# mit-han-lab/duo-attention

Measured on NVIDIA H100. Metric: decode tok/s @512K ctx (+ prefill tok/s @128K in `prefill`), Llama-3-8B, DuoAttention 50% retrieval heads, higher is better.
Workload: dtype bf16

## Files before the change

### duo_attention_b200/csrc/attn_tc.cu

```cuda
#include <cstdlib>

#include "duo_common.cuh"

namespace duo {

constexpr int TC_THREADS = 384;
constexpr int TC_TILE = 128;
constexpr int TC_BOX_BYTES = TC_TILE * 128;
constexpr int TC_TILE_BYTES = 2 * TC_BOX_BYTES;
constexpr int TC_MAX_W = kTcMaxWindow;
constexpr int TC_SMEM_BYTES = 5 * TC_TILE_BYTES + TC_MAX_W + 1024;

struct TcParams {
  void* out;
  long long out_batch_stride;
  int q_len, n_q_heads, group, n_full, n_stream, batch;
  int sink, recent, W;
  long long full_len, total, lo;
  float scale_log2;
  int cache_scan;
  int n_tok_tiles;
  int seq_rank, seq_world, seq_block;
  float* part_o;
  float* part_lse;
};

__device__ __forceinline__ void wg_fence() { asm volatile("wgmma.fence.sync.aligned;" ::: "memory"); }
__device__ __forceinline__ void wg_commit() { asm volatile("wgmma.commit_group.sync.aligned;" ::: "memory"); }
template <int N>
__device__ __forceinline__ void wg_wait() {
  asm volatile("wgmma.wait_group.sync.aligned %0;" ::"n"(N) : "memory");
}
__device__ __forceinline__ void wg_fence_regs(float (&d)[64]) {
#pragma unroll
  for (int i = 0; i < 64; ++i) asm volatile("" : "+f"(d[i])::"memory");
}

__device__ __forceinline__ uint64_t make_smem_desc(uint32_t saddr, uint32_t lbo_bytes, uint32_t sbo_bytes) {
  uint64_t d = 0;
  d |= (uint64_t)((saddr >> 4) & 0x3FFF);
  d |= (uint64_t)((lbo_bytes >> 4) & 0x3FFF) << 16;
  d |= (uint64_t)((sbo_bytes >> 4) & 0x3FFF) << 32;
  d |= 1ull << 62;
  return d;
}

template <bool BF16>
__device__ __forceinline__ void wgmma_ss(float (&d)[64], uint64_t adesc, uint64_t bdesc, uint32_t accum) {
  if constexpr (BF16) {
    asm volatile(
        "{\n\t.reg .pred p;\n\tsetp.ne.b32 p, %66, 0;\n\t"
        "wgmma.mma_async.sync.aligned.m64n128k16.f32.bf16.bf16 {%0,%1,%2,%3,%4,%5,%6,%7,%8,%9,%10,%11,%12,%13,%14,%15,%16,%17,%18,%19,%20,%21,%22,%23,%24,%25,%26,%27,%28,%29,%30,%31,%32,%33,%34,%35,%36,%37,%38,%39,%40,%41,%42,%43,%44,%45,%46,%47,%48,%49,%50,%51,%52,%53,%54,%55,%56,%57,%58,%59,%60,%61,%62,%63}, %64, %65, p, 1, 1, 0, 0;\n\t}"
        : "+f"(d[0]), "+f"(d[1]), "+f"(d[2]), "+f"(d[3]), "+f"(d[4]), "+f"(d[5]), "+f"(d[6]), "+f"(d[7]), "+f"(d[8]), "+f"(d[9]), "+f"(d[10]), "+f"(d[11]), "+f"(d[12]), "+f"(d[13]), "+f"(d[14]), "+f"(d[15]), "+f"(d[16]), "+f"(d[17]), "+f"(d[18]), "+f"(d[19]), "+f"(d[20]), "+f"(d[21]), "+f"(d[22]), "+f"(d[23]), "+f"(d[24]), "+f"(d[25]), "+f"(d[26]), "+f"(d[27]), "+f"(d[28]), "+f"(d[29]), "+f"(d[30]), "+f"(d[31]), "+f"(d[32]), "+f"(d[33]), "+f"(d[34]), "+f"(d[35]), "+f"(d[36]), "+f"(d[37]), "+f"(d[38]), "+f"(d[39]), "+f"(d[40]), "+f"(d[41]), "+f"(d[42]), "+f"(d[43]), "+f"(d[44]), "+f"(d[45]), "+f"(d[46]), "+f"(d[47]), "+f"(d[48]), "+f"(d[49]), "+f"(d[50]), "+f"(d[51]), "+f"(d[52]), "+f"(d[53]), "+f"(d[54]), "+f"(d[55]), "+f"(d[56]), "+f"(d[57]), "+f"(d[58]), "+f"(d[59]), "+f"(d[60]), "+f"(d[61]), "+f"(d[62]), "+f"(d[63])
        : "l"(adesc), "l"(bdesc), "r"(accum));
  } else {
    asm volatile(
        "{\n\t.reg .pred p;\n\tsetp.ne.b32 p, %66, 0;\n\t"
        "wgmma.mma_async.sync.aligned.m64n128k16.f32.f16.f16 {%0,%1,%2,%3,%4,%5,%6,%7,%8,%9,%10,%11,%12,%13,%14,%15,%16,%17,%18,%19,%20,%21,%22,%23,%24,%25,%26,%27,%28,%29,%30,%31,%32,%33,%34,%35,%36,%37,%38,%39,%40,%41,%42,%43,%44,%45,%46,%47,%48,%49,%50,%51,%52,%53,%54,%55,%56,%57,%58,%59,%60,%61,%62,%63}, %64, %65, p, 1, 1, 0, 0;\n\t}"
        : "+f"(d[0]), "+f"(d[1]), "+f"(d[2]), "+f"(d[3]), "+f"(d[4]), "+f"(d[5]), "+f"(d[6]), "+f"(d[7]), "+f"(d[8]), "+f"(d[9]), "+f"(d[10]), "+f"(d[11]), "+f"(d[12]), "+f"(d[13]), "+f"(d[14]), "+f"(d[15]), "+f"(d[16]), "+f"(d[17]), "+f"(d[18]), "+f"(d[19]), "+f"(d[20]), "+f"(d[21]), "+f"(d[22]), "+f"(d[23]), "+f"(d[24]), "+f"(d[25]), "+f"(d[26]), "+f"(d[27]), "+f"(d[28]), "+f"(d[29]), "+f"(d[30]), "+f"(d[31]), "+f"(d[32]), "+f"(d[33]), "+f"(d[34]), "+f"(d[35]), "+f"(d[36]), "+f"(d[37]), "+f"(d[38]), "+f"(d[39]), "+f"(d[40]), "+f"(d[41]), "+f"(d[42]), "+f"(d[43]), "+f"(d[44]), "+f"(d[45]), "+f"(d[46]), "+f"(d[47]), "+f"(d[48]), "+f"(d[49]), "+f"(d[50]), "+f"(d[51]), "+f"(d[52]), "+f"(d[53]), "+f"(d[54]), "+f"(d[55]), "+f"(d[56]), "+f"(d[57]), "+f"(d[58]), "+f"(d[59]), "+f"(d[60]), "+f"(d[61]), "+f"(d[62]), "+f"(d[63])
        : "l"(adesc), "l"(bdesc), "r"(accum));
  }
}
template <bool BF16>
__device__ __forceinline__ void wgmma_rs(float (&d)[64], const uint32_t* a, uint64_t bdesc) {
  if constexpr (BF16) {
    asm volatile(
        "{\n\t.reg .pred p;\n\tsetp.ne.b32 p, %69, 0;\n\t"
        "wgmma.mma_async.sync.aligned.m64n128k16.f32.bf16.bf16 {%0,%1,%2,%3,%4,%5,%6,%7,%8,%9,%10,%11,%12,%13,%14,%15,%16,%17,%18,%19,%20,%21,%22,%23,%24,%25,%26,%27,%28,%29,%30,%31,%32,%33,%34,%35,%36,%37,%38,%39,%40,%41,%42,%43,%44,%45,%46,%47,%48,%49,%50,%51,%52,%53,%54,%55,%56,%57,%58,%59,%60,%61,%62,%63}, {%64, %65, %66, %67}, %68, p, 1, 1, 1;\n\t}"
        : "+f"(d[0]), "+f"(d[1]), "+f"(d[2]), "+f"(d[3]), "+f"(d[4]), "+f"(d[5]), "+f"(d[6]), "+f"(d[7]), "+f"(d[8]), "+f"(d[9]), "+f"(d[10]), "+f"(d[11]), "+f"(d[12]), "+f"(d[13]), "+f"(d[14]), "+f"(d[15]), "+f"(d[16]), "+f"(d[17]), "+f"(d[18]), "+f"(d[19]), "+f"(d[20]), "+f"(d[21]), "+f"(d[22]), "+f"(d[23]), "+f"(d[24]), "+f"(d[25]), "+f"(d[26]), "+f"(d[27]), "+f"(d[28]), "+f"(d[29]), "+f"(d[30]), "+f"(d[31]), "+f"(d[32]), "+f"(d[33]), "+f"(d[34]), "+f"(d[35]), "+f"(d[36]), "+f"(d[37]), "+f"(d[38]), "+f"(d[39]), "+f"(d[40]), "+f"(d[41]), "+f"(d[42]), "+f"(d[43]), "+f"(d[44]), "+f"(d[45]), "+f"(d[46]), "+f"(d[47]), "+f"(d[48]), "+f"(d[49]), "+f"(d[50]), "+f"(d[51]), "+f"(d[52]), "+f"(d[53]), "+f"(d[54]), "+f"(d[55]), "+f"(d[56]), "+f"(d[57]), "+f"(d[58]), "+f"(d[59]), "+f"(d[60]), "+f"(d[61]), "+f"(d[62]), "+f"(d[63])
        : "r"(a[0]), "r"(a[1]), "r"(a[2]), "r"(a[3]), "l"(bdesc), "r"(1));
  } else {
    asm volatile(
        "{\n\t.reg .pred p;\n\tsetp.ne.b32 p, %69, 0;\n\t"
        "wgmma.mma_async.sync.aligned.m64n128k16.f32.f16.f16 {%0,%1,%2,%3,%4,%5,%6,%7,%8,%9,%10,%11,%12,%13,%14,%15,%16,%17,%18,%19,%20,%21,%22,%23,%24,%25,%26,%27,%28,%29,%30,%31,%32,%33,%34,%35,%36,%37,%38,%39,%40,%41,%42,%43,%44,%45,%46,%47,%48,%49,%50,%51,%52,%53,%54,%55,%56,%57,%58,%59,%60,%61,%62,%63}, {%64, %65, %66, %67}, %68, p, 1, 1, 1;\n\t}"
        : "+f"(d[0]), "+f"(d[1]), "+f"(d[2]), "+f"(d[3]), "+f"(d[4]), "+f"(d[5]), "+f"(d[6]), "+f"(d[7]), "+f"(d[8]), "+f"(d[9]), "+f"(d[10]), "+f"(d[11]), "+f"(d[12]), "+f"(d[13]), "+f"(d[14]), "+f"(d[15]), "+f"(d[16]), "+f"(d[17]), "+f"(d[18]), "+f"(d[19]), "+f"(d[20]), "+f"(d[21]), "+f"(d[22]), "+f"(d[23]), "+f"(d[24]), "+f"(d[25]), "+f"(d[26]), "+f"(d[27]), "+f"(d[28]), "+f"(d[29]), "+f"(d[30]), "+f"(d[31]), "+f"(d[32]), "+f"(d[33]), "+f"(d[34]), "+f"(d[35]), "+f"(d[36]), "+f"(d[37]), "+f"(d[38]), "+f"(d[39]), "+f"(d[40]), "+f"(d[41]), "+f"(d[42]), "+f"(d[43]), "+f"(d[44]), "+f"(d[45]), "+f"(d[46]), "+f"(d[47]), "+f"(d[48]), "+f"(d[49]), "+f"(d[50]), "+f"(d[51]), "+f"(d[52]), "+f"(d[53]), "+f"(d[54]), "+f"(d[55]), "+f"(d[56]), "+f"(d[57]), "+f"(d[58]), "+f"(d[59]), "+f"(d[60]), "+f"(d[61]), "+f"(d[62]), "+f"(d[63])
        : "r"(a[0]), "r"(a[1]), "r"(a[2]), "r"(a[3]), "l"(bdesc), "r"(1));
  }
}

template <typename T>
struct TcType;
template <>
struct TcType<__nv_bfloat16> {
  static constexpr bool bf16 = true;
  __device__ static uint32_t pack(float a, float b) {
    __nv_bfloat162 v = __floats2bfloat162_rn(a, b);
    return *reinterpret_cast<uint32_t*>(&v);
  }
};
template <>
struct TcType<__half> {
  static constexpr bool bf16 = false;
  __device__ static uint32_t pack(float a, float b) {
    __half2 v = __floats2half2_rn(a, b);
    return *reinterpret_cast<uint32_t*>(&v);
  }
};

struct TcBarriers {
  uint64_t q_full;
  uint64_t k_full[2], k_empty[2], v_full[2], v_empty[2];
};

template <typename T, bool SEQ = false, bool SHARE = false, bool RAGGED = false>
__global__ void __launch_bounds__(TC_THREADS, 1)
duo_attn_tc_kernel(const __grid_constant__ CUtensorMap map_q, const __grid_constant__ CUtensorMap map_fk,
                   const __grid_constant__ CUtensorMap map_fv, const __grid_constant__ CUtensorMap map_rk,
                   const __grid_constant__ CUtensorMap map_rv, const TcParams p,
                   const __grid_constant__ CUtensorMap map_pk, const __grid_constant__ CUtensorMap map_pv,
                   const long long share_len, const __grid_constant__ RaggedChunks rc) {
  static_assert(!(SEQ && SHARE), "a shared prefix is not sequence-sharded");
  static_assert(!(RAGGED && (SEQ || SHARE)), "a ragged prefill reads sharing from row_share, and is not sharded");
  extern __shared__ __align__(1024) uint8_t smem_raw[];
  uint8_t* smem = reinterpret_cast<uint8_t*>((reinterpret_cast<uintptr_t>(smem_raw) + 1023) & ~uintptr_t(1023));
  __shared__ TcBarriers bars;

  uint8_t* sQ = smem;
  uint8_t* sK = smem + 1 * TC_TILE_BYTES;
  uint8_t* sV = smem + 3 * TC_TILE_BYTES;
  uint8_t* sValid = smem + 5 * TC_TILE_BYTES;

  const int tid = threadIdx.x;
  const int b = blockIdx.y;

  int x = blockIdx.x;
  const int per_kvh = p.group * p.n_tok_tiles;
  const int kvh = x / per_kvh;
  x -= kvh * per_kvh;
  const int qh = kvh * p.group + x / p.n_tok_tiles;
  int q_len = p.q_len, n_tok_tiles = p.n_tok_tiles, cache_scan = p.cache_scan, q_off = 0, donor = -1;
  long long full_len = p.full_len, total = p.total, lo = p.lo, pre_len = 0;
  if constexpr (RAGGED) {
    q_len = rc.len[b];
    n_tok_tiles = (q_len + TC_TILE - 1) / TC_TILE;
    if (x % p.n_tok_tiles >= n_tok_tiles) return;
    q_off = rc.off[b];
    full_len = rc.row_state[4 * b];
    total = rc.row_state[4 * b + 1];
    lo = rc.row_state[4 * b + 2];
    cache_scan = (int)min((long long)p.W, total);
    pre_len = ragged_chunk_share(rc, b, donor);
  }
  const int tok0 = (n_tok_tiles - 1 - (x % p.n_tok_tiles)) * TC_TILE;
  const bool is_full = kvh < p.n_full;
  const int tok_hi = min(q_len, tok0 + TC_TILE);
  long long a0 = 0, a1, b0 = 0, b1 = 0, base;
  if (is_full) {
    base = full_len;
    a1 = full_len + tok_hi;
    if constexpr (SEQ) a1 = seq_local_len(a1, p.seq_rank, p.seq_world, p.seq_block);
  } else {
    base = p.W;
    a1 = cache_scan;
    b0 = p.W;
    b1 = (long long)p.W + tok_hi;
  }
  const int nA = (int)((a1 - a0 + TC_TILE - 1) / TC_TILE);
  const int nB = (int)((b1 - b0 + TC_TILE - 1) / TC_TILE);
  const int n_tiles = nA + nB;
  const CUtensorMap* mk = is_full ? &map_fk : &map_rk;
  const CUtensorMap* mv = is_full ? &map_fv : &map_rv;
  const int head_coord = is_full ? (b * p.n_full + kvh) : (b * p.n_stream + (kvh - p.n_full));
  auto tile_start = [&](int i) -> long long {
    return i < nA ? a0 + (long long)i * TC_TILE : b0 + (long long)(i - nA) * TC_TILE;
  };

  if (tid == 0) {
    prefetch_tmap(&map_q);
    prefetch_tmap(mk);
    prefetch_tmap(mv);
    if constexpr (SHARE) {
      if (is_full) {
        prefetch_tmap(&map_pk);
        prefetch_tmap(&map_pv);
      }
    }
    mbar_init(&bars.q_full, 1);
    for (int s = 0; s < 2; ++s) {
      mbar_init(&bars.k_full[s], 1);
      mbar_init(&bars.k_empty[s], 256);
      mbar_init(&bars.v_full[s], 1);
      mbar_init(&bars.v_empty[s], 256);
    }
    fence_barrier_init();
  }
  if (!is_full) {
    for (int j = tid; j < p.W; j += TC_THREADS) sValid[j] = stream_slot_valid(j, p.sink, p.recent, total, lo) ? 1 : 0;
  }
  __syncthreads();

  if (tid < 128) {
    asm volatile("setmaxnreg.dec.sync.aligned.u32 24;");
    if constexpr (SEQ) {
      if (n_tiles == 0) return;
    }
    if (tid == 0) {
      mbar_expect_tx(&bars.q_full, TC_TILE_BYTES);
      const int q_row = RAGGED ? q_off + tok0 : tok0, q_b = RAGGED ? 0 : b;
      tma_load_3d(sQ, &map_q, &bars.q_full, qh * kHeadDim, q_row, q_b);
      tma_load_3d(sQ + TC_BOX_BYTES, &map_q, &bars.q_full, qh * kHeadDim + 64, q_row, q_b);
      for (int j = 0; j < n_tiles; ++j) {
        const int st = j & 1;
        const uint32_t ph = (j >> 1) & 1;
        if constexpr (RAGGED) {
          const long long t0 = tile_start(j);
          int r0 = (int)t0, hc = head_coord;
          if (is_full && rc.row_geom) {
            const bool pre = t0 < pre_len;
            r0 = (int)(pre ? ragged_pool_row(rc, donor, p.n_full, kvh, t0) : ragged_pool_row(rc, b, p.n_full, kvh, t0 - pre_len));
            hc = 0;
          }
          mbar_wait(&bars.k_empty[st], ph ^ 1);
          mbar_expect_tx(&bars.k_full[st], TC_TILE_BYTES);
          tma_load_3d(sK + st * TC_TILE_BYTES, mk, &bars.k_full[st], 0, r0, hc);
          tma_load_3d(sK + st * TC_TILE_BYTES + TC_BOX_BYTES, mk, &bars.k_full[st], 64, r0, hc);
          mbar_wait(&bars.v_empty[st], ph ^ 1);
          mbar_expect_tx(&bars.v_full[st], TC_TILE_BYTES);
          tma_load_3d(sV + st * TC_TILE_BYTES, mv, &bars.v_full[st], 0, r0, hc);
          tma_load_3d(sV + st * TC_TILE_BYTES + TC_BOX_BYTES, mv, &bars.v_full[st], 64, r0, hc);
          continue;
        }
        if constexpr (SHARE) {
          const long long t0 = tile_start(j);
          const bool pre = is_full && t0 < share_len;
          const CUtensorMap* tk = pre ? &map_pk : mk;
          const CUtensorMap* tv = pre ? &map_pv : mv;
          const int r0 = (int)(is_full && !pre ? t0 - share_len : t0);
          mbar_wait(&bars.k_empty[st], ph ^ 1);
          mbar_expect_tx(&bars.k_full[st], TC_TILE_BYTES);
          tma_load_3d(sK + st * TC_TILE_BYTES, tk, &bars.k_full[st], 0, r0, head_coord);
          tma_load_3d(sK + st * TC_TILE_BYTES + TC_BOX_BYTES, tk, &bars.k_full[st], 64, r0, head_coord);
          mbar_wait(&bars.v_empty[st], ph ^ 1);
          mbar_expect_tx(&bars.v_full[st], TC_TILE_BYTES);
          tma_load_3d(sV + st * TC_TILE_BYTES, tv, &bars.v_full[st], 0, r0, head_coord);
          tma_load_3d(sV + st * TC_TILE_BYTES + TC_BOX_BYTES, tv, &bars.v_full[st], 64, r0, head_coord);
          continue;
        }
        const int j0 = (int)tile_start(j);
        mbar_wait(&bars.k_empty[st], ph ^ 1);
        mbar_expect_tx(&bars.k_full[st], TC_TILE_BYTES);
        tma_load_3d(sK + st * TC_TILE_BYTES, mk, &bars.k_full[st], 0, j0, head_coord);
        tma_load_3d(sK + st * TC_TILE_BYTES + TC_BOX_BYTES, mk, &bars.k_full[st], 64, j0, head_coord);
        mbar_wait(&bars.v_empty[st], ph ^ 1);
        mbar_expect_tx(&bars.v_full[st], TC_TILE_BYTES);
        tma_load_3d(sV + st * TC_TILE_BYTES, mv, &bars.v_full[st], 0, j0, head_coord);
        tma_load_3d(sV + st * TC_TILE_BYTES + TC_BOX_BYTES, mv, &bars.v_full[st], 64, j0, head_coord);
      }
    }
    return;
  }

  asm volatile("setmaxnreg.inc.sync.aligned.u32 240;");
  constexpr bool kBf16 = TcType<T>::bf16;
  const int wg = (tid >> 7) - 1;
  const int wt = tid & 127;
  const int quad = wt & 3;
  const int row0 = wg * 64 + (wt >> 5) * 16 + ((wt & 31) >> 2);
  const float c = p.scale_log2;
  long long min_limit = base + tok0 + wg * 64;
  int tok[2];
  bool row_ok[2];
  long long limit[2];
#pragma unroll
  for (int i = 0; i < 2; ++i) {
    tok[i] = tok0 + row0 + 8 * i;
    row_ok[i] = tok[i] < q_len;
    limit[i] = base + tok[i];
  }
  auto seq_last_key = [&](int t) { return seq_local_len(p.full_len + t + 1, p.seq_rank, p.seq_world, p.seq_block) - 1; };
  if constexpr (SEQ) {
    if (is_full) {
      min_limit = seq_last_key(tok0 + wg * 64);
#pragma unroll
      for (int i = 0; i < 2; ++i) limit[i] = seq_last_key(tok[i]);
    }
  }

  const uint32_t q_addr = smem_u32(sQ) + wg * 64 * 128, k_addr = smem_u32(sK), v_addr = smem_u32(sV);
  auto issue_s = [&](float (&s)[64], int st) {
    const uint32_t ka = k_addr + st * TC_TILE_BYTES;
#pragma unroll
    for (int kk = 0; kk < 8; ++kk) {
      const uint32_t off = (kk >> 2) * TC_BOX_BYTES + (kk & 3) * 32;
      wgmma_ss<kBf16>(s, make_smem_desc(q_addr + off, 16, 1024), make_smem_desc(ka + off, 16, 1024), kk > 0);
    }
  };
  auto issue_pv = [&](float (&o)[64], const uint32_t (&pk)[32], int st) {
    const uint32_t va = v_addr + st * TC_TILE_BYTES;
#pragma unroll
    for (int kk = 0; kk < 8; ++kk) wgmma_rs<kBf16>(o, &pk[4 * kk], make_smem_desc(va + kk * 2048, TC_BOX_BYTES, 1024));
  };

  float s[64], o[64];
#pragma unroll
  for (int i = 0; i < 64; ++i) o[i] = 0.f;
  float m_run[2] = {-INFINITY, -INFINITY};
  float l_run[2] = {0.f, 0.f};

  auto store_partial = [&](int i, float inv, float l) {
    if (!row_ok[i]) return;
    const long long row = ((long long)b * p.q_len + tok[i]) * p.n_q_heads + qh;
#pragma unroll
    for (int nb = 0; nb < 16; ++nb)
      *reinterpret_cast<float2*>(p.part_o + row * kHeadDim + nb * 8 + quad * 2) =
          make_float2(o[nb * 4 + 2 * i] * inv, o[nb * 4 + 2 * i + 1] * inv);
    if (quad == 0) p.part_lse[row] = l > 0.f ? m_run[i] * c + log2f(l) : -INFINITY;
  };
  if constexpr (SEQ) {
    if (n_tiles == 0) {
      store_partial(0, 0.f, 0.f);
      store_partial(1, 0.f, 0.f);
      return;
    }
  }
  mbar_wait(&bars.q_full, 0);
  mbar_wait(&bars.k_full[0], 0);
  wg_fence();
  issue_s(s, 0);
  wg_commit();
  wg_wait<0>();
  wg_fence_regs(s);
  mbar_arrive(&bars.k_empty[0]);

  for (int j = 0; j < n_tiles; ++j) {
    const int st = j & 1;
    const uint32_t ph = (j >> 1) & 1;
    const long long j0 = tile_start(j);
    const long long jend = (j < nA) ? a1 : b1;
    const bool cache_seg = (!is_full) && (j < nA);
    const bool need_mask = cache_seg || (j0 + TC_TILE > jend) || (j0 + TC_TILE - 1 > min_limit);
    if (need_mask) {
#pragma unroll
      for (int nb = 0; nb < 16; ++nb) {
#pragma unroll
        for (int e = 0; e < 2; ++e) {
          const long long jj = j0 + nb * 8 + quad * 2 + e;
          bool slot_ok = jj < jend;
          if (cache_seg) slot_ok = slot_ok && (jj < p.W) && (sValid[jj < p.W ? jj : 0] != 0);
#pragma unroll
          for (int i = 0; i < 2; ++i)
            if (!(slot_ok && row_ok[i] && jj <= limit[i])) s[nb * 4 + 2 * i + e] = -INFINITY;
        }
      }
    }
    uint32_t pk[32];
#pragma unroll
    for (int i = 0; i < 2; ++i) {
      float mx = -INFINITY;
#pragma unroll
      for (int nb = 0; nb < 16; ++nb) mx = fmaxf(mx, fmaxf(s[nb * 4 + 2 * i], s[nb * 4 + 2 * i + 1]));
      mx = fmaxf(mx, __shfl_xor_sync(0xffffffffu, mx, 1));
      mx = fmaxf(mx, __shfl_xor_sync(0xffffffffu, mx, 2));
      const float m_new = fmaxf(m_run[i], mx);
      const float alpha = (m_new == -INFINITY) ? 1.f : fast_exp2((m_run[i] - m_new) * c);
      const float mref_c = (m_new == -INFINITY) ? 0.f : m_new * c;
      m_run[i] = m_new;
      float rs = 0.f;
#pragma unroll
      for (int nb = 0; nb < 16; ++nb) {
        const float p0 = fast_exp2(__fmaf_rn(s[nb * 4 + 2 * i], c, -mref_c));
        const float p1 = fast_exp2(__fmaf_rn(s[nb * 4 + 2 * i + 1], c, -mref_c));
        rs += p0 + p1;
        pk[nb * 2 + i] = TcType<T>::pack(p0, p1);
        o[nb * 4 + 2 * i] *= alpha;
        o[nb * 4 + 2 * i + 1] *= alpha;
      }
      l_run[i] = l_run[i] * alpha + rs;
    }
    mbar_wait_spin(&bars.v_full[st], ph);
    wg_fence();
    issue_pv(o, pk, st);
    wg_commit();
    const bool more = j + 1 < n_tiles;
    if (more) {
      const int st1 = (j + 1) & 1;
      mbar_wait_spin(&bars.k_full[st1], ((j + 1) >> 1) & 1);
      wg_fence();
      issue_s(s, st1);
      wg_commit();
    }
    wg_wait<0>();
    wg_fence_regs(o);
    wg_fence_regs(s);
    mbar_arrive(&bars.v_empty[st]);
    if (more) mbar_arrive(&bars.k_empty[(j + 1) & 1]);
  }

  if constexpr (SEQ) {
    if (is_full) {
#pragma unroll
      for (int i = 0; i < 2; ++i) {
        float l = l_run[i];
        l += __shfl_xor_sync(0xffffffffu, l, 1);
        l += __shfl_xor_sync(0xffffffffu, l, 2);
        store_partial(i, l > 0.f ? 1.f / l : 0.f, l);
      }
      return;
    }
  }
  T* out_b = reinterpret_cast<T*>(p.out) + (RAGGED ? (long long)q_off * p.n_q_heads * kHeadDim : (long long)b * p.out_batch_stride);
#pragma unroll
  for (int i = 0; i < 2; ++i) {
    float l = l_run[i];
    l += __shfl_xor_sync(0xffffffffu, l, 1);
    l += __shfl_xor_sync(0xffffffffu, l, 2);
    const float inv = l > 0.f ? 1.f / l : 0.f;
    if (row_ok[i]) {
      T* dst = out_b + ((long long)tok[i] * p.n_q_heads + qh) * kHeadDim + quad * 2;
#pragma unroll
      for (int nb = 0; nb < 16; ++nb)
        *reinterpret_cast<uint32_t*>(dst + nb * 8) = TcType<T>::pack(o[nb * 4 + 2 * i] * inv, o[nb * 4 + 2 * i + 1] * inv);
    }
  }
}

typedef CUresult (*EncodeTiledFn)(CUtensorMap*, CUtensorMapDataType, cuuint32_t, void*, const cuuint64_t*,
                                  const cuuint64_t*, const cuuint32_t*, const cuuint32_t*, CUtensorMapInterleave,
                                  CUtensorMapSwizzle, CUtensorMapL2promotion, CUtensorMapFloatOOBfill);
EncodeTiledFn get_encode_fn();

bool tc_prefill_supported(const duo_layer* L, const duo_cache_state* st, int q_len) {
  (void)st;
  if (L->d.kv_format != DUO_KV_SAME) return false;
  if (q_len < TC_TILE) return false;
  if (L->d.sink + L->d.recent > TC_MAX_W) return false;
  return true;
}

template <bool SEQ, bool SHARE = false>
static int launch_tc(const duo_layer* L, const duo_cache_state* st, const void* q, long long q_row_stride, void* out,
                     float* part_o, float* part_lse, int q_len, float scale, cudaStream_t stream,
                     const duo_layer* prefix = nullptr, long long share_len = 0) {
  const duo_layer_desc& d = L->d;
  EncodeTiledFn fn = get_encode_fn();
  if (!fn) return DUO_ECUDA;
  CUtensorMap map_q;
  {
    cuuint64_t dims[3] = {(cuuint64_t)q_row_stride, (cuuint64_t)q_len, (cuuint64_t)d.batch};
    cuuint64_t strides[2] = {(cuuint64_t)q_row_stride * 2, (cuuint64_t)q_row_stride * 2 * (cuuint64_t)q_len};
    cuuint32_t box[3] = {64, TC_TILE, 1};
    cuuint32_t estr[3] = {1, 1, 1};
    CUresult r = fn(&map_q, d.dtype == DUO_DT_BF16 ? CU_TENSOR_MAP_DATA_TYPE_BFLOAT16 : CU_TENSOR_MAP_DATA_TYPE_FLOAT16, 3,
                    const_cast<void*>(q), dims, strides, box, estr, CU_TENSOR_MAP_INTERLEAVE_NONE,
                    CU_TENSOR_MAP_SWIZZLE_128B, CU_TENSOR_MAP_L2_PROMOTION_L2_256B, CU_TENSOR_MAP_FLOAT_OOB_FILL_NONE);
    if (r != CUDA_SUCCESS) {
      set_error("cuTensorMapEncodeTiled(q) failed with CUresult %d", (int)r);
      return DUO_ECUDA;
    }
  }
  TcParams p{};
  p.out = out;
  const int n_q = (d.n_full + d.n_stream) * d.group;
  p.out_batch_stride = (long long)q_len * n_q * kHeadDim;
  p.q_len = q_len;
  p.n_q_heads = n_q;
  p.group = d.group;
  p.n_full = d.n_full;
  p.n_stream = d.n_stream;
  p.batch = d.batch;
  p.sink = d.sink;
  p.recent = d.recent;
  p.W = d.sink + d.recent;
  p.full_len = st->full_len;
  p.total = st->total;
  p.lo = st->lo;
  p.scale_log2 = scale * 1.4426950408889634f;
  p.cache_scan = (int)std::min<long long>(p.W, st->total);
  p.n_tok_tiles = (q_len + TC_TILE - 1) / TC_TILE;
  p.seq_rank = st->seq_rank;
  p.seq_world = st->seq_world;
  p.seq_block = st->seq_block;
  p.part_o = part_o;
  p.part_lse = part_lse;
  const dim3 grid(n_q * p.n_tok_tiles, d.batch);
  const KvMaps m = kv_maps(L, true);
  const KvMaps pm = kv_maps(SHARE ? prefix : L, true);
  return dispatch_dtype(d.dtype, [&](auto t) {
    auto kern = duo_attn_tc_kernel<decltype(t), SEQ, SHARE>;
    static unsigned long long attr_mask = 0;
    if (int rc = ensure_dyn_smem(kern, TC_SMEM_BYTES, &attr_mask)) return rc;
    kern<<<grid, TC_THREADS, TC_SMEM_BYTES, stream>>>(map_q, *m.fk, *m.fv, *m.rk, *m.rv, p, *pm.fk, *pm.fv, share_len,
                                                      RaggedChunks{});
    DUO_CUDA_TRY(cudaGetLastError());
    return DUO_OK;
  });
}

int launch_rope_append_ragged(const duo_layer* L, const RaggedChunks& rc, void* qkv, long long row_stride,
                              const void* cos, const void* sin, int rope_mode, cudaStream_t stream);
int launch_stream_commit_ragged(const duo_layer* L, const RaggedChunks& rc, cudaStream_t stream);

int launch_prefill_ragged(const duo_layer* L, const RaggedChunks& rc, void* qkv, long long row_stride, const void* cos,
                          const void* sin, int rope_mode, void* out, float scale, cudaStream_t stream) {
  const duo_layer_desc& d = L->d;
  const int n_tok = rc.off[rc.batch];
  int max_tiles = 0;
  for (int b = 0; b < rc.batch; ++b) max_tiles = std::max(max_tiles, (rc.len[b] + TC_TILE - 1) / TC_TILE);
  if (n_tok == 0) return DUO_OK;
  EncodeTiledFn fn = get_encode_fn();
  if (!fn) return DUO_ECUDA;
  CUtensorMap map_q;
  {
    cuuint64_t dims[3] = {(cuuint64_t)row_stride, (cuuint64_t)n_tok, 1};
    cuuint64_t strides[2] = {(cuuint64_t)row_stride * 2, (cuuint64_t)row_stride * 2 * (cuuint64_t)n_tok};
    cuuint32_t box[3] = {64, TC_TILE, 1};
    cuuint32_t estr[3] = {1, 1, 1};
    CUresult r = fn(&map_q, d.dtype == DUO_DT_BF16 ? CU_TENSOR_MAP_DATA_TYPE_BFLOAT16 : CU_TENSOR_MAP_DATA_TYPE_FLOAT16, 3,
                    qkv, dims, strides, box, estr, CU_TENSOR_MAP_INTERLEAVE_NONE, CU_TENSOR_MAP_SWIZZLE_128B,
                    CU_TENSOR_MAP_L2_PROMOTION_L2_256B, CU_TENSOR_MAP_FLOAT_OOB_FILL_NONE);
    if (r != CUDA_SUCCESS) {
      set_error("cuTensorMapEncodeTiled(q) failed with CUresult %d", (int)r);
      return DUO_ECUDA;
    }
  }
  TcParams p{};
  p.out = out;
  const int n_q = (d.n_full + d.n_stream) * d.group;
  p.n_q_heads = n_q;
  p.group = d.group;
  p.n_full = d.n_full;
  p.n_stream = d.n_stream;
  p.batch = d.batch;
  p.sink = d.sink;
  p.recent = d.recent;
  p.W = d.sink + d.recent;
  p.scale_log2 = scale * 1.4426950408889634f;
  p.n_tok_tiles = max_tiles;
  const dim3 grid(n_q * max_tiles, d.batch);
  const KvMaps m = kv_maps(L, true);
  return dispatch_dtype(d.dtype, [&](auto t) {
    auto kern = duo_attn_tc_kernel<decltype(t), false, false, true>;
    static unsigned long long attr_mask = 0;
    if (int rc2 = ensure_dyn_smem(kern, TC_SMEM_BYTES, &attr_mask)) return rc2;
    if (int rc2 = launch_rope_append_ragged(L, rc, qkv, row_stride, cos, sin, rope_mode, stream)) return rc2;
    kern<<<grid, TC_THREADS, TC_SMEM_BYTES, stream>>>(map_q, *m.fk, *m.fv, *m.rk, *m.rv, p, *m.fk, *m.fv, 0, rc);
    DUO_CUDA_TRY(cudaGetLastError());
    return launch_stream_commit_ragged(L, rc, stream);
  });
}

int launch_attn_tc(const duo_layer* L, const duo_cache_state* st, const void* q, long long q_row_stride, void* out,
                   int q_len, float scale, cudaStream_t stream) {
  return launch_tc<false>(L, st, q, q_row_stride, out, nullptr, nullptr, q_len, scale, stream);
}

int launch_attn_tc_seq(const duo_layer* L, const duo_cache_state* st, const void* q, long long q_row_stride, void* out,
                       float* part_o, float* part_lse, int q_len, float scale, cudaStream_t stream) {
  return launch_tc<true>(L, st, q, q_row_stride, out, part_o, part_lse, q_len, scale, stream);
}

int launch_attn_tc_shared(const duo_layer* L, const duo_layer* prefix, long long share_len, const duo_cache_state* st,
                          const void* q, long long q_row_stride, void* out, int q_len, float scale, cudaStream_t stream) {
  return launch_tc<false, true>(L, st, q, q_row_stride, out, nullptr, nullptr, q_len, scale, stream, prefix, share_len);
}

}
```

Baseline: 58.17.

## Overlap softmax of next tile with in-flight PV wgmma in attention loop

Restructures the tensor-core attention main loop so that after issuing QK^T for tile j+1 and PV for tile j, it waits only for the S result and computes the softmax of tile j+1 while the PV wgmma is still executing. P packing and O rescaling move into a separate step, and the O rescale is skipped when every alpha in the warp equals one. This hides softmax latency behind the tensor cores, at the cost of extra register pressure from keeping P in s and pk at the same time. Decode at 512K context is probably dominated by memory bandwidth, so the benefit there may be limited. The change mostly targets prefill.

```diff
diff --git a/duo_attention_b200/csrc/attn_tc.cu b/duo_attention_b200/csrc/attn_tc.cu
--- a/duo_attention_b200/csrc/attn_tc.cu
+++ b/duo_attention_b200/csrc/attn_tc.cu
@@ -34,6 +34,11 @@
 __device__ __forceinline__ void wg_fence_regs(float (&d)[64]) {
 #pragma unroll
   for (int i = 0; i < 64; ++i) asm volatile("" : "+f"(d[i])::"memory");
+}
+
+__device__ __forceinline__ void wg_fence_pk(uint32_t (&a)[32]) {
+#pragma unroll
+  for (int i = 0; i < 32; ++i) asm volatile("" : "+r"(a[i])::"memory");
 }
 
 __device__ __forceinline__ uint64_t make_smem_desc(uint32_t saddr, uint32_t lbo_bytes, uint32_t sbo_bytes) {
@@ -313,6 +318,67 @@
       return;
     }
   }
+  float alpha[2];
+  auto softmax = [&](int j) {
+    const long long j0 = tile_start(j);
+    const long long jend = (j < nA) ? a1 : b1;
+    const bool cache_seg = (!is_full) && (j < nA);
+    const bool need_mask = cache_seg || (j0 + TC_TILE > jend) || (j0 + TC_TILE - 1 > min_limit);
+    if (need_mask) {
+#pragma unroll
+      for (int nb = 0; nb < 16; ++nb) {
+#pragma unroll
+        for (int e = 0; e < 2; ++e) {
+          const long long jj = j0 + nb * 8 + quad * 2 + e;
+          bool slot_ok = jj < jend;
+          if (cache_seg) slot_ok = slot_ok && (jj < p.W) && (sValid[jj < p.W ? jj : 0] != 0);
+#pragma unroll
+          for (int i = 0; i < 2; ++i)
+            if (!(slot_ok && row_ok[i] && jj <= limit[i])) s[nb * 4 + 2 * i + e] = -INFINITY;
+        }
+      }
+    }
+#pragma unroll
+    for (int i = 0; i < 2; ++i) {
+      float mx = -INFINITY;
+#pragma unroll
+      for (int nb = 0; nb < 16; ++nb) mx = fmaxf(mx, fmaxf(s[nb * 4 + 2 * i], s[nb * 4 + 2 * i + 1]));
+      mx = fmaxf(mx, __shfl_xor_sync(0xffffffffu, mx, 1));
+      mx = fmaxf(mx, __shfl_xor_sync(0xffffffffu, mx, 2));
+      const float m_new = fmaxf(m_run[i], mx);
+      alpha[i] = (m_new == -INFINITY) ? 1.f : fast_exp2((m_run[i] - m_new) * c);
+      const float mref_c = (m_new == -INFINITY) ? 0.f : m_new * c;
+      m_run[i] = m_new;
+      float rs = 0.f;
+#pragma unroll
+      for (int nb = 0; nb < 16; ++nb) {
+        const float p0 = fast_exp2(__fmaf_rn(s[nb * 4 + 2 * i], c, -mref_c));
+        const float p1 = fast_exp2(__fmaf_rn(s[nb * 4 + 2 * i + 1], c, -mref_c));
+        rs += p0 + p1;
+        s[nb * 4 + 2 * i] = p0;
+        s[nb * 4 + 2 * i + 1] = p1;
+      }
+      l_run[i] = l_run[i] * alpha[i] + rs;
+    }
+  };
+  uint32_t pk[32];
+  auto finish_p = [&] {
+#pragma unroll
+    for (int nb = 0; nb < 16; ++nb)
+#pragma unroll
+      for (int i = 0; i < 2; ++i) pk[nb * 2 + i] = TcType<T>::pack(s[nb * 4 + 2 * i], s[nb * 4 + 2 * i + 1]);
+    if (__any_sync(0xffffffffu, alpha[0] != 1.f || alpha[1] != 1.f)) {
+#pragma unroll
+      for (int nb = 0; nb < 16; ++nb) {
+#pragma unroll
+        for (int i = 0; i < 2; ++i) {
+          o[nb * 4 + 2 * i] *= alpha[i];
+          o[nb * 4 + 2 * i + 1] *= alpha[i];
+        }
+      }
+    }
+  };
+
   mbar_wait(&bars.q_full, 0);
   mbar_wait(&bars.k_full[0], 0);
   wg_fence();
@@ -321,69 +387,37 @@
   wg_wait<0>();
   wg_fence_regs(s);
   mbar_arrive(&bars.k_empty[0]);
-
-  for (int j = 0; j < n_tiles; ++j) {
-    const int st = j & 1;
-    const uint32_t ph = (j >> 1) & 1;
-    const long long j0 = tile_start(j);
-    const long long jend = (j < nA) ? a1 : b1;
-    const bool cache_seg = (!is_full) && (j < nA);
-    const bool need_mask = cache_seg || (j0 + TC_TILE > jend) || (j0 + TC_TILE - 1 > min_limit);
-    if (need_mask) {
-#pragma unroll
-      for (int nb = 0; nb < 16; ++nb) {
-#pragma unroll
-        for (int e = 0; e < 2; ++e) {
-          const long long jj = j0 + nb * 8 + quad * 2 + e;
-          bool slot_ok = jj < jend;
-          if (cache_seg) slot_ok = slot_ok && (jj < p.W) && (sValid[jj < p.W ? jj : 0] != 0);
-#pragma unroll
-          for (int i = 0; i < 2; ++i)
-            if (!(slot_ok && row_ok[i] && jj <= limit[i])) s[nb * 4 + 2 * i + e] = -INFINITY;
-        }
-      }
-    }
-    uint32_t pk[32];
-#pragma unroll
-    for (int i = 0; i < 2; ++i) {
-      float mx = -INFINITY;
-#pragma unroll
-      for (int nb = 0; nb < 16; ++nb) mx = fmaxf(mx, fmaxf(s[nb * 4 + 2 * i], s[nb * 4 + 2 * i + 1]));
-      mx = fmaxf(mx, __shfl_xor_sync(0xffffffffu, mx, 1));
-      mx = fmaxf(mx, __shfl_xor_sync(0xffffffffu, mx, 2));
-      const float m_new = fmaxf(m_run[i], mx);
-      const float alpha = (m_new == -INFINITY) ? 1.f : fast_exp2((m_run[i] - m_new) * c);
-      const float mref_c = (m_new == -INFINITY) ? 0.f : m_new * c;
-      m_run[i] = m_new;
-      float rs = 0.f;
-#pragma unroll
-      for (int nb = 0; nb < 16; ++nb) {
-        const float p0 = fast_exp2(__fmaf_rn(s[nb * 4 + 2 * i], c, -mref_c));
-        const float p1 = fast_exp2(__fmaf_rn(s[nb * 4 + 2 * i + 1], c, -mref_c));
-        rs += p0 + p1;
-        pk[nb * 2 + i] = TcType<T>::pack(p0, p1);
-        o[nb * 4 + 2 * i] *= alpha;
-        o[nb * 4 + 2 * i + 1] *= alpha;
-      }
-      l_run[i] = l_run[i] * alpha + rs;
-    }
-    mbar_wait_spin(&bars.v_full[st], ph);
+  softmax(0);
+
+  for (int j = 0; j + 1 < n_tiles; ++j) {
+    const int st = j & 1, st1 = (j + 1) & 1;
+    finish_p();
+    mbar_wait_spin(&bars.v_full[st], (j >> 1) & 1);
+    mbar_wait_spin(&bars.k_full[st1], ((j + 1) >> 1) & 1);
+    wg_fence();
+    issue_s(s, st1);
+    wg_commit();
+    issue_pv(o, pk, st);
+    wg_commit();
+    wg_wait<1>();
+    wg_fence_regs(s);
+    mbar_arrive(&bars.k_empty[st1]);
+    softmax(j + 1);
+    wg_wait<0>();
+    wg_fence_regs(o);
+    wg_fence_pk(pk);
+    mbar_arrive(&bars.v_empty[st]);
+  }
+  {
+    const int j = n_tiles - 1, st = j & 1;
+    finish_p();
+    mbar_wait_spin(&bars.v_full[st], (j >> 1) & 1);
     wg_fence();
     issue_pv(o, pk, st);
     wg_commit();
-    const bool more = j + 1 < n_tiles;
-    if (more) {
-      const int st1 = (j + 1) & 1;
-      mbar_wait_spin(&bars.k_full[st1], ((j + 1) >> 1) & 1);
-      wg_fence();
-      issue_s(s, st1);
-      wg_commit();
-    }
     wg_wait<0>();
     wg_fence_regs(o);
-    wg_fence_regs(s);
     mbar_arrive(&bars.v_empty[st]);
-    if (more) mbar_arrive(&bars.k_empty[(j + 1) & 1]);
   }
 
   if constexpr (SEQ) {
```

Result: no change. 58.15, median of 6 (-0.0%).

## Overlap softmax with PV wgmma and ping-pong warpgroups via named barriers

Applied to the files above, without the earlier changes.

Restructures the tensor-core attention main loop in FA3 style. The softmax of tile j+1 now runs while the PV wgmma of tile j is in flight (wait_group 1), and O rescaling is skipped when no row max changed. The two consumer warpgroups also take turns issuing wgmma through named bar.sync/bar.arrive barriers, so one group's softmax overlaps the other's matmuls. This adds register pressure (pk is kept alive across iterations) and barrier-protocol complexity, and the main benefit is in prefill rather than in memory-bound decode.

```diff
diff --git a/duo_attention_b200/csrc/attn_tc.cu b/duo_attention_b200/csrc/attn_tc.cu
--- a/duo_attention_b200/csrc/attn_tc.cu
+++ b/duo_attention_b200/csrc/attn_tc.cu
@@ -34,6 +34,10 @@
 __device__ __forceinline__ void wg_fence_regs(float (&d)[64]) {
 #pragma unroll
   for (int i = 0; i < 64; ++i) asm volatile("" : "+f"(d[i])::"memory");
+}
+__device__ __forceinline__ void wg_fence_regs(uint32_t (&a)[32]) {
+#pragma unroll
+  for (int i = 0; i < 32; ++i) asm volatile("" : "+r"(a[i])::"memory");
 }
 
 __device__ __forceinline__ uint64_t make_smem_desc(uint32_t saddr, uint32_t lbo_bytes, uint32_t sbo_bytes) {
@@ -313,18 +317,8 @@
       return;
     }
   }
-  mbar_wait(&bars.q_full, 0);
-  mbar_wait(&bars.k_full[0], 0);
-  wg_fence();
-  issue_s(s, 0);
-  wg_commit();
-  wg_wait<0>();
-  wg_fence_regs(s);
-  mbar_arrive(&bars.k_empty[0]);
-
-  for (int j = 0; j < n_tiles; ++j) {
-    const int st = j & 1;
-    const uint32_t ph = (j >> 1) & 1;
+  float alpha[2];
+  auto softmax = [&](int j) {
     const long long j0 = tile_start(j);
     const long long jend = (j < nA) ? a1 : b1;
     const bool cache_seg = (!is_full) && (j < nA);
@@ -343,7 +337,6 @@
         }
       }
     }
-    uint32_t pk[32];
 #pragma unroll
     for (int i = 0; i < 2; ++i) {
       float mx = -INFINITY;
@@ -352,7 +345,7 @@
       mx = fmaxf(mx, __shfl_xor_sync(0xffffffffu, mx, 1));
       mx = fmaxf(mx, __shfl_xor_sync(0xffffffffu, mx, 2));
       const float m_new = fmaxf(m_run[i], mx);
-      const float alpha = (m_new == -INFINITY) ? 1.f : fast_exp2((m_run[i] - m_new) * c);
+      alpha[i] = (m_new == -INFINITY) ? 1.f : fast_exp2((m_run[i] - m_new) * c);
       const float mref_c = (m_new == -INFINITY) ? 0.f : m_new * c;
       m_run[i] = m_new;
       float rs = 0.f;
@@ -361,29 +354,87 @@
         const float p0 = fast_exp2(__fmaf_rn(s[nb * 4 + 2 * i], c, -mref_c));
         const float p1 = fast_exp2(__fmaf_rn(s[nb * 4 + 2 * i + 1], c, -mref_c));
         rs += p0 + p1;
-        pk[nb * 2 + i] = TcType<T>::pack(p0, p1);
-        o[nb * 4 + 2 * i] *= alpha;
-        o[nb * 4 + 2 * i + 1] *= alpha;
+        s[nb * 4 + 2 * i] = p0;
+        s[nb * 4 + 2 * i + 1] = p1;
       }
-      l_run[i] = l_run[i] * alpha + rs;
-    }
-    mbar_wait_spin(&bars.v_full[st], ph);
+      l_run[i] = l_run[i] * alpha[i] + rs;
+    }
+  };
+  auto rescale_o = [&] {
+    if (!__any_sync(0xffffffffu, alpha[0] != 1.f || alpha[1] != 1.f)) return;
+#pragma unroll
+    for (int nb = 0; nb < 16; ++nb) {
+#pragma unroll
+      for (int i = 0; i < 2; ++i) {
+        o[nb * 4 + 2 * i] *= alpha[i];
+        o[nb * 4 + 2 * i + 1] *= alpha[i];
+      }
+    }
+  };
+  uint32_t pk[32];
+  auto pack_p = [&] {
+#pragma unroll
+    for (int nb = 0; nb < 16; ++nb) {
+#pragma unroll
+      for (int i = 0; i < 2; ++i) pk[nb * 2 + i] = TcType<T>::pack(s[nb * 4 + 2 * i], s[nb * 4 + 2 * i + 1]);
+    }
+  };
+  const int my_turn = 1 + wg, their_turn = 2 - wg;
+  int turns_left = n_tiles + 1;
+  auto take_turn = [&] { asm volatile("bar.sync %0, 256;" ::"r"(my_turn) : "memory"); };
+  auto pass_turn = [&] {
+    if (--turns_left > 0 || wg == 0) asm volatile("bar.arrive %0, 256;" ::"r"(their_turn) : "memory");
+  };
+  if (wg == 0) asm volatile("bar.arrive %0, 256;" ::"r"(my_turn) : "memory");
+
+  mbar_wait(&bars.q_full, 0);
+  mbar_wait(&bars.k_full[0], 0);
+  take_turn();
+  wg_fence();
+  issue_s(s, 0);
+  wg_commit();
+  pass_turn();
+  wg_wait<0>();
+  wg_fence_regs(s);
+  mbar_arrive(&bars.k_empty[0]);
+  softmax(0);
+  pack_p();
+
+  for (int j = 0; j + 1 < n_tiles; ++j) {
+    const int st = j & 1, st1 = (j + 1) & 1;
+    mbar_wait_spin(&bars.k_full[st1], ((j + 1) >> 1) & 1);
+    mbar_wait_spin(&bars.v_full[st], (j >> 1) & 1);
+    take_turn();
+    wg_fence();
+    issue_s(s, st1);
+    wg_commit();
+    rescale_o();
     wg_fence();
     issue_pv(o, pk, st);
     wg_commit();
-    const bool more = j + 1 < n_tiles;
-    if (more) {
-      const int st1 = (j + 1) & 1;
-      mbar_wait_spin(&bars.k_full[st1], ((j + 1) >> 1) & 1);
-      wg_fence();
-      issue_s(s, st1);
-      wg_commit();
-    }
+    pass_turn();
+    wg_wait<1>();
+    wg_fence_regs(s);
+    mbar_arrive(&bars.k_empty[st1]);
+    softmax(j + 1);
     wg_wait<0>();
     wg_fence_regs(o);
-    wg_fence_regs(s);
+    wg_fence_regs(pk);
     mbar_arrive(&bars.v_empty[st]);
-    if (more) mbar_arrive(&bars.k_empty[(j + 1) & 1]);
+    pack_p();
+  }
+  {
+    const int j = n_tiles - 1;
+    mbar_wait_spin(&bars.v_full[j & 1], (j >> 1) & 1);
+    take_turn();
+    rescale_o();
+    wg_fence();
+    issue_pv(o, pk, j & 1);
+    wg_commit();
+    pass_turn();
+    wg_wait<0>();
+    wg_fence_regs(o);
+    mbar_arrive(&bars.v_empty[j & 1]);
   }
 
   if constexpr (SEQ) {
```

Result: no change. 58.44 before, 58.37 after (median of 6 runs) (-0.1%).
